# snap-research/GiGL

Measured on AMD Instinct MI355X. Metric: sampled+aggregated edges/s, higher is better.
Workload: dtype f32

## Files before the change

### gigl_amd/csrc/sample.hip

```cpp
#include "common.h"

#include <cstdlib>
#include <mutex>
#include <type_traits>

namespace {

constexpr uint64_t P1 = 0x9E3779B185EBCA87ULL;
constexpr uint64_t P2 = 0xC2B2AE3D27D4EB4FULL;
constexpr uint64_t P3 = 0x165667B19E3779F9ULL;
constexpr uint64_t P5 = 0x27D4EB2F165667C5ULL;
constexpr uint64_t SPARK_SEED = 42ULL;
constexpr uint64_t SIGN = 0x8000000000000000ULL;

__device__ __forceinline__ uint64_t xxh64_i32_ordered(uint32_t x) {
  uint64_t h = (SPARK_SEED + P5 + 4ULL) ^ ((uint64_t)x * P1);
  h = ((h << 23) | (h >> 41)) * P2 + P3;
  h ^= h >> 33;
  h *= P2;
  h ^= h >> 29;
  h *= P3;
  h ^= h >> 32;
  return h ^ SIGN;
}
// ... 373 lines not shown
    }
    return finish(count, lk, li);
  }
  __device__ __forceinline__ void serial(const RangeTable& tb, uint32_t n, uint32_t base, uint32_t T, bool in_table) {
    reset_best();
    if (!in_table) {
      scan_row(nullptr, (int64_t)n, base);
      return;
    }
    const uint32_t T4 = T >= (1u << 30) ? 0xFFFFFFFFu : 4u * T;
    const int l4 = T4 == 0xFFFFFFFFu ? 0 : min((int)__builtin_clz(T4 - 1u), tb.levels);
    if (l4 > 0) {
      if (scan_level(tb, l4, T4, n, base)) return;
      reset_best();
    }
    if constexpr (FAST) {
      scan_row(tb.flat, (int64_t)n, base);
      if (readlane32(idx, f - 1) == 0xFFFFFFFFu) tie = true;
    } else {
      scan_row(nullptr, (int64_t)n, base);
    }
  }
};

enum { ROW_INVALID = 0, ROW_COPY = 1, ROW_FLAT = 2, ROW_LEVEL = 3, ROW_HASH = 4, ROW_SERIAL = 5, ROW_SERIAL_HASH = 6,
       ROW_SKIP = 7 };

struct __attribute__((aligned(32))) RowDesc {
  int64_t s;
  uint32_t n;
  uint32_t base;
  uint32_t T;
  uint32_t kind_cnt;
  const void* ptr;
};

__device__ __forceinline__ float filter_lambda(int f) { return (float)f + 4.f * __builtin_sqrtf((float)f) + 4.f; }

constexpr int WORK_LISTS = 64;
constexpr int WORK_CNT_STRIDE = 32;

struct WorkLists {
  uint32_t* items;
  int32_t* count;
  int64_t cap;
  int32_t iters;
  int32_t wgs;
};

__host__ __device__ static inline int64_t work_list_cap(int64_t n_parents) {
  return ((n_parents / 256 + 1 + WORK_LISTS - 1) / WORK_LISTS) * 256;
}
static inline int64_t expand_desc_bytes(int64_t n_parents) {
  return (n_parents + 1) * (int64_t)sizeof(RowDesc) + WORK_LISTS * work_list_cap(n_parents) * 4 +
         WORK_LISTS * WORK_CNT_STRIDE * 4 + 512;
}

__global__ void work_counts_zero_kernel(int32_t* count) { count[threadIdx.x * WORK_CNT_STRIDE] = 0; }

__global__ __launch_bounds__(256) void plan_rows_kernel(ExpandArgs a, RangeTable tb, RowDesc* __restrict__ desc,
                                                        int64_t* heavy_list, int32_t* heavy_count, WorkLists wl) {
  __shared__ int32_t s_wave[4];
  __shared__ int32_t s_base;
  const uint32_t p = blockIdx.x * 256u + threadIdx.x;
  const int lane = threadIdx.x & 63, w = threadIdx.x >> 6;
  bool real = false;
  if (p <= (uint32_t)a.n_parents) {
    RowDesc d{};
    if (p == (uint32_t)a.n_parents) {
      d.kind_cnt = ROW_SKIP;
      desc[p] = d;
    } else {
      uint32_t v, ksum;
      parent_of(a, p, v, ksum);
      uint32_t* out = a.out_nbr + (int64_t)p * a.f;
      if (v == GIGL_INVALID || (int64_t)v >= a.n_nodes) {
        for (int j = 0; j < a.f; ++j) out[j] = GIGL_INVALID;
        a.out_cnt[p] = 0;
      } else {
        int64_t deg;
        if (a.peer_world) {
          const uint32_t q = v / a.peer_world, rk = v - q * a.peer_world;
          const int64_t* rp = a.peer_rowptr[rk];
          const int64_t s0 = rp[q];
          deg = rp[q + 1] - s0;
          d.s = ((int64_t)rk << 48) | s0;
        } else {
          d.s = a.rowptr[v];
          deg = a.rowptr[v + 1] - d.s;
        }
        d.n = (uint32_t)deg;
        d.base = ksum + (uint32_t)a.hash_add;
        if (deg <= a.f && !a.multi) {
          const uint32_t* row = row_of_desc(a, d.s);
          for (int j = 0; j < a.f; ++j) out[j] = j < (int)deg ? row[j] : GIGL_INVALID;
          a.out_cnt[p] = (int32_t)deg;
        } else if (deg <= a.f) {
          d.kind_cnt = ROW_COPY;
          desc[p] = d;
          real = true;
        } else {
          const bool in_table = (uint64_t)d.base + (uint64_t)deg < tb.dom;
          const float lam = filter_lambda(a.f);
          d.T = d.n <= 64u ? 0xFFFFFFFFu
                           : (uint32_t)fminf(lam * 4294967296.f * __builtin_amdgcn_rcpf((float)d.n), 4294967040.f);
          uint32_t kind;
          if (!in_table) {
            if (deg > HEAVY_DEG) {
              kind = ROW_SKIP;
              if (heavy_list) heavy_list[atomicAdd(heavy_count, 1)] = (int64_t)p;
            } else {
              kind = lam <= 56.f ? ROW_HASH : ROW_SERIAL_HASH;
            }
          } else if (lam > 56.f) {
            kind = ROW_SERIAL;
          } else {
            const int l = min((int)__builtin_clz(d.T - 1u), tb.levels);
            if (l == 0 || d.n <= (uint32_t)a.flat_max) {
              kind = ROW_FLAT;
              d.ptr = tb.flat;
            } else {
              const int gs = TBL_IDX_SHIFT + l;
              const uint32_t* off = tb.off[l];
              const uint32_t start = off[(d.base + 1u) >> gs], end = off[((d.base + d.n) >> gs) + 1u];
              if (end - start > 256u) {
                kind = ROW_SERIAL;
              } else {
                kind = ROW_LEVEL | ((end - start) << 3);
                d.ptr = tb.lvl[l] + start;
              }
            }
          }
          d.kind_cnt = kind;
          desc[p] = d;
          real = (kind & 7u) != ROW_SKIP;
        }
      }
    }
  }
  const unsigned long long m = __ballot(real);
  if (lane == 0) s_wave[w] = (int32_t)__popcll(m);
  __syncthreads();
  const int list = (int)(blockIdx.x % WORK_LISTS);
  if (threadIdx.x == 0) {
    const int32_t tot = s_wave[0] + s_wave[1] + s_wave[2] + s_wave[3];
    s_base = tot ? atomicAdd(&wl.count[list * WORK_CNT_STRIDE], tot) : 0;
  }
  __syncthreads();
  if (real) {
    int32_t pos = s_base + (int32_t)__popcll(m & ((1ull << lane) - 1ull));
    for (int k = 0; k < w; ++k) pos += s_wave[k];
    wl.items[(int64_t)list * wl.cap + pos] = p;
  }
}

struct Cand {
  uint32_t k0, j0, k1, j1;
  bool ahead;
};

__device__ __forceinline__ Cand fetch_candidates(const RowDesc& d, int lane) {
  Cand c;
  c.k0 = c.k1 = 0xFFFFFFFFu;
  c.j0 = c.j1 = d.base;
  c.ahead = false;
  const uint32_t kind = d.kind_cnt & 7u, cnt = d.kind_cnt >> 3;
  if (kind == ROW_LEVEL && cnt <= 128u) {
    const uint2* ent = (const uint2*)d.ptr;
    if ((uint32_t)lane < cnt) {
      const uint2 x = ent[lane];
      c.j0 = x.x;
      c.k0 = x.y;
    }
    if ((uint32_t)lane + 64u < cnt) {
      const uint2 x = ent[lane + 64];
      c.j1 = x.x;
      c.k1 = x.y;
    }
    c.ahead = true;
  } else if (kind == ROW_FLAT && d.n <= 128u) {
    const uint32_t* src = (const uint32_t*)d.ptr + d.base;
    c.j0 = d.base + (uint32_t)lane + 1u;
    c.k0 = src[lane + 1];
    if (d.n > 64u) {
      c.j1 = c.j0 + 64u;
      c.k1 = src[lane + 65];
    }
    c.ahead = true;
  }
  return c;
}

__device__ __forceinline__ bool select_ahead(Sel<true>& sel, const RowDesc& d, const Cand& c, uint32_t* lk, uint32_t* li) {
  const uint32_t n = d.n, T = d.T, base = d.base;
  const bool all = T == 0xFFFFFFFFu;
  uint32_t count = 0;
  const uint32_t i0 = c.j0 - base, i1 = c.j1 - base;
  sel.offer(c.k0 & sel.dmask, i0, (uint32_t)(i0 - 1u) < n && (all || c.k0 < T), count, lk, li);
  if ((d.kind_cnt & 7u) == ROW_LEVEL ? (d.kind_cnt >> 3) > 64u : n > 64u)
    sel.offer(c.k1 & sel.dmask, i1, (uint32_t)(i1 - 1u) < n && (all || c.k1 < T), count, lk, li);
  return sel.finish(count, lk, li);
}

__global__ __launch_bounds__(256) __attribute__((amdgpu_waves_per_eu(8, 8))) void expand_rows_kernel(
    ExpandArgs a, RangeTable tb, const RowDesc* __restrict__ desc, WorkLists wl) {
  __shared__ __attribute__((aligned(16))) uint32_t s_lk[4][72], s_li[4][64];
  const int lane = threadIdx.x & 63;
  const int wave_in_block = __builtin_amdgcn_readfirstlane((int)(threadIdx.x >> 6));
  const int f = a.f;
  uint32_t* lk = s_lk[wave_in_block];
  uint32_t* li = s_li[wave_in_block];
  const uint32_t wgs_p = wl.iters > 0 ? (uint32_t)wl.wgs : gridDim.x;
  const uint32_t round = blockIdx.x / wgs_p;
  const uint32_t gw = (blockIdx.x % wgs_p) * 4u + (uint32_t)wave_in_block, n_waves = wgs_p * 4u;
  const uint32_t list = gw % WORK_LISTS, stride = n_waves / WORK_LISTS;
  const int32_t n_items = __builtin_amdgcn_readfirstlane(wl.count[list * WORK_CNT_STRIDE]);
  const uint32_t* items = wl.items + (int64_t)list * wl.cap;
  const uint32_t k_first = gw / WORK_LISTS + stride * round * (uint32_t)wl.iters;
  const uint32_t k_end = wl.iters > 0 ? k_first + stride * (uint32_t)wl.iters : 0xFFFFFFFFu;
  for (uint32_t k = k_first; (int32_t)(2u * k) < n_items && k < k_end; k += stride) {
    const uint32_t p0 = __builtin_amdgcn_readfirstlane(items[2u * k]);
    const uint32_t p1 = (int32_t)(2u * k + 1u) < n_items ? __builtin_amdgcn_readfirstlane(items[2u * k + 1u])
                                                         : (uint32_t)a.n_parents;
    const RowDesc d0 = desc[p0], d1 = desc[p1];
    const Cand c0 = fetch_candidates(d0, lane), c1 = fetch_candidates(d1, lane);
    Sel<true> s0, s1;
    s0.init(f, lane, a.proxy_drop);
    s1.init(f, lane, a.proxy_drop);
    const bool done0 = c0.ahead && !a.multi && select_ahead(s0, d0, c0, lk, li) && !s0.tie;
    uint32_t slot0 = 0, val0 = 0;
    bool sel0 = false;
    if (done0) {
      const unsigned long long m = s0.selmask;
      sel0 = (m >> lane) & 1ull;
      slot0 = __builtin_amdgcn_mbcnt_hi((uint32_t)(m >> 32), __builtin_amdgcn_mbcnt_lo((uint32_t)m, 0u));
      if (sel0) val0 = row_of_desc(a, d0.s)[s0.idx - 1];
    }
    const bool done1 = c1.ahead && !a.multi && select_ahead(s1, d1, c1, lk, li) && !s1.tie;
    uint32_t slot1 = 0, val1 = 0;
    bool sel1 = false;
    if (done1) {
      const unsigned long long m = s1.selmask;
      sel1 = (m >> lane) & 1ull;
      slot1 = __builtin_amdgcn_mbcnt_hi((uint32_t)(m >> 32), __builtin_amdgcn_mbcnt_lo((uint32_t)m, 0u));
      if (sel1) val1 = row_of_desc(a, d1.s)[s1.idx - 1];
    }
    if (done0) {
      if (sel0) a.out_nbr[(int64_t)p0 * f + slot0] = val0;
      if (lane == 0) a.out_cnt[p0] = f;
    }
    if (done1) {
      if (sel1) a.out_nbr[(int64_t)p1 * f + slot1] = val1;
      if (lane == 0) a.out_cnt[p1] = f;
    }
    if (done0 && done1) continue;
  #pragma nounroll
    for (int r = 0; r < 2; ++r) {
      if (r == 0 ? done0 : done1) continue;
      const RowDesc d = r == 0 ? d0 : d1;
      const uint32_t p = r == 0 ? p0 : p1;
      const uint32_t kind = d.kind_cnt & 7u;
      if (kind == ROW_SKIP) continue;
      uint32_t* out = a.out_nbr + (int64_t)p * f;
      if (kind == ROW_INVALID) {
        if (lane < f) out[lane] = GIGL_INVALID;
        if (lane == 0) a.out_cnt[p] = 0;
        continue;
      }
      const uint32_t* row = row_of_desc(a, d.s);
      const uint32_t n = d.n, base = d.base, T = d.T;
      if (kind == ROW_COPY) {
        if (a.multi) {
          const int nw = emit_sorted_distinct(row, (uint32_t)lane < n ? (uint32_t)lane + 1u : 0xFFFFFFFFu, f, lane, out);
          if (lane == 0) a.out_cnt[p] = nw;
          continue;
        }
        if (lane < f) out[lane] = (uint32_t)lane < n ? row[lane] : GIGL_INVALID;
        if (lane == 0) a.out_cnt[p] = (int32_t)n;
        continue;
      }
      const bool in_table = kind != ROW_HASH && kind != ROW_SERIAL_HASH;
      uint32_t sel_idx;
      {
        Sel<true> fast;
        fast.init(f, lane, a.proxy_drop);
        bool done = false;
        if (kind == ROW_LEVEL) done = fast.filter_level((const uint2*)d.ptr, d.kind_cnt >> 3, n, T, base, lk, li);
        else if (kind == ROW_FLAT) done = fast.template filter_positions<SRC_FLAT>((const uint32_t*)d.ptr, n, T, base, lk, li);
        else if (kind == ROW_HASH) done = fast.template filter_positions<SRC_HASH>(nullptr, n, T, base, lk, li);
        if (!done) fast.serial(tb, n, base, T, in_table);
        sel_idx = fast.idx;
        if (fast.tie) {
          Sel<false> exact;
          exact.init(f, lane);
          exact.serial(tb, n, base, T, in_table);
          sel_idx = exact.idx;
        } else if (fast.ordered) {
          const unsigned long long m = fast.selmask;
          const bool sel = (m >> lane) & 1ull;
          const uint32_t slot = __builtin_amdgcn_mbcnt_hi((uint32_t)(m >> 32), __builtin_amdgcn_mbcnt_lo((uint32_t)m, 0u));
          const uint32_t val = sel ? row[sel_idx - 1] : GIGL_INVALID;
          if (!a.multi) {
            if (sel) out[slot] = val;
            if (lane == 0) a.out_cnt[p] = f;
            continue;
          }
          if (sel) lk[slot] = val;
          wave_lds_sync();
          const bool keep = sel && (slot == 0 || lk[slot - 1] != val);
          wave_lds_sync();
          const unsigned long long km = __ballot(keep);
          if (lane < f) out[lane] = GIGL_INVALID;
          if (keep) out[__builtin_amdgcn_mbcnt_hi((uint32_t)(km >> 32), __builtin_amdgcn_mbcnt_lo((uint32_t)km, 0u))] = val;
          if (lane == 0) a.out_cnt[p] = (int32_t)__popcll(km);
          continue;
        }
      }
      if (a.multi) {
        const int nw = emit_sorted_distinct(row, sel_idx, f, lane, out);
        if (lane == 0) a.out_cnt[p] = nw;
        continue;
      }
      emit_sorted(row, sel_idx, f, lane, out);
// ... 384 lines not shown
  e = hipMalloc(&own->mem2, bytes2);
  if (e != hipSuccess) {
    own->mem2 = nullptr;
    return fail_build(GIGL_E_OOM, "hipMalloc of the level lists failed", e);
  }
  RangeTable t{};
  t.dom = dom;
  t.levels = L;
  t.flat = flat;
  TableBuild tbuild{};
  tbuild.flat = flat;
  tbuild.tile_off = cnt;
  tbuild.total = total;
  tbuild.n_tiles = n_tiles;
  tbuild.levels = L;
  tbuild.dom = dom;
  for (int l = 1; l <= L; ++l) {
    tbuild.lvl[l] = (uint2*)((char*)own->mem2 + lvl_at[l]);
    tbuild.off[l] = (uint32_t*)(m0 + off_at[l]);
    t.lvl[l] = tbuild.lvl[l];
    t.off[l] = tbuild.off[l];
  }
  hipLaunchKernelGGL(table_fill_kernel, dim3(n_tiles), dim3(256), 0, ctx->stream, tbuild);
  e = hipGetLastError();
  if (e == hipSuccess) e = hipStreamSynchronize(ctx->stream);
  if (e != hipSuccess) return fail_build(GIGL_E_HIP, "filling failed", e);
  own->t = t;
  own->refs = 1;
  g_device_table[dev] = own;
  ctx->sampler_table = own;
  return GIGL_OK;
}

int32_t run_expand(gigl_ctx* ctx, const ExpandArgs& a_in, const RangeTable& tb, bool covered,
                   int64_t* heavy_list, int32_t* heavy_count, RowDesc* desc) {
  ExpandArgs a = a_in;
  if (a.f > GIGL_FAST_FANOUT) {
    gigl_prof_scope ps(ctx, GIGL_K_EXPAND);
    int64_t wgs = a.n_parents < 8192 ? a.n_parents : 8192;
    hipLaunchKernelGGL(expand_wide_kernel, dim3((unsigned)wgs), dim3(256), 0, ctx->stream, a);
    GIGL_HIP_CHECK(ctx, hipGetLastError());
    return GIGL_OK;
  }
  a.proxy_drop = 0;
  if (const char* e = getenv("GIGL_SAMPLER_PROXY_BITS")) {
    int bits = atoi(e);
    if (bits >= 1 && bits <= 32) a.proxy_drop = 32 - bits;
  }
  static const int32_t flat_max = [] {
    const char* e = getenv("GIGL_EXPAND_FLAT_MAX");
    return e ? atoi(e) : 128;
  }();
  a.flat_max = flat_max;
  if (!covered) gigl_fill_u32(ctx->stream, heavy_count, 0u, 1);
  WorkLists wl{};
  wl.cap = work_list_cap(a.n_parents);
  wl.items = reinterpret_cast<uint32_t*>(desc + a.n_parents + 1);
  wl.count = reinterpret_cast<int32_t*>(wl.items + (int64_t)WORK_LISTS * wl.cap);
  wl.count = reinterpret_cast<int32_t*>(((uintptr_t)wl.count + 127) & ~(uintptr_t)127);
  hipLaunchKernelGGL(work_counts_zero_kernel, dim3(1), dim3(WORK_LISTS), 0, ctx->stream, wl.count);
  {
    gigl_prof_scope ps(ctx, GIGL_K_EXPAND);
    hipLaunchKernelGGL(plan_rows_kernel, dim3((unsigned)(a.n_parents / 256 + 1)), dim3(256), 0, ctx->stream, a, tb,
                       desc, covered ? nullptr : heavy_list, heavy_count, wl);
    int64_t wgs = ((a.n_parents + 7) / 8 + 15) / 16 * 16;
    static const int64_t wgs_max = [] {
      const char* e = getenv("GIGL_EXPAND_WGS");
      const int64_t v = e ? atoll(e) : 2048;
      return v < 16 ? (int64_t)16 : v / 16 * 16;
    }();
    if (wgs > wgs_max) wgs = wgs_max;
    static const int32_t iters = [] {
      const char* e = getenv("GIGL_EXPAND_ITERS");
      const int v = e ? atoi(e) : 16;
      return v < 0 ? 0 : v;
    }();
    wl.iters = iters;
    wl.wgs = (int32_t)wgs;
    if (iters > 0) {
      const int64_t stride = wgs * 4 / WORK_LISTS;
      const int64_t steps = (wl.cap / 2 + stride - 1) / stride;
      wgs *= (steps + iters - 1) / iters;
    }
    hipLaunchKernelGGL(expand_rows_kernel, dim3((unsigned)wgs), dim3(256), 0, ctx->stream, a, tb, (const RowDesc*)desc, wl);
  }
  if (!covered) {
    gigl_prof_scope ps(ctx, GIGL_K_EXPAND_HEAVY);
    int64_t hb = a.n_parents < 2048 ? a.n_parents : 2048;
    hipLaunchKernelGGL(expand_heavy_kernel, dim3((unsigned)hb), dim3(256), 0, ctx->stream, a, heavy_list,
                       heavy_count);
  }
  GIGL_HIP_CHECK(ctx, hipGetLastError());
  return GIGL_OK;
}

uint64_t window_bound(const gigl_graph* g, int32_t hops, int32_t first_counter, int32_t sampling_seed) {
  uint64_t worst = 0;
  for (int k = 0; k < hops; ++k) {
    int64_t add = (int64_t)sampling_seed * (int64_t)(first_counter + k);
    if (add < 0 || add > (int64_t)0x7FFFFFFF) return ~0ULL;
    uint64_t hi = (uint64_t)(k + 1) * (uint64_t)(g->n > 0 ? g->n - 1 : 0) + (uint64_t)add + (uint64_t)g->maxdeg;
    if (hi > worst) worst = hi;
  }
  return worst;
}

__device__ __forceinline__ uint32_t mix32(uint32_t x) {
  x ^= x >> 16;
  x *= 0x7feb352dU;
  x ^= x >> 15;
  x *= 0x846ca68bU;
  x ^= x >> 16;
  return x;
}

__global__ __launch_bounds__(256) void expand_fast_kernel(ExpandArgs a) {
  const int lane = threadIdx.x & 63;
// ... 84 lines not shown
               "bad mode %d", mode);
  int64_t parents = b;
  for (int k = 0; k < hops; ++k) {
    if (fanouts[k] < 1 || fanouts[k] > GIGL_MAX_FANOUT)
      return gigl_fail(ctx, GIGL_E_UNSUPPORTED, "fanout[%d]=%d outside [1,%d]", k, fanouts[k],
                       GIGL_MAX_FANOUT);
    if (mode != GIGL_MODE_SPARK_HASH && fanouts[k] > GIGL_FAST_FANOUT)
      return gigl_fail(ctx, GIGL_E_UNSUPPORTED, "fanout[%d]=%d: the non-parity modes take fanouts up to %d", k, fanouts[k],
                       GIGL_FAST_FANOUT);
    GIGL_REQUIRE(ctx, out->nbr[k] && out->cnt[k], "tree buffers for hop %d are null", k);
    parents *= fanouts[k];
    GIGL_REQUIRE(ctx, parents < (int64_t)1 << 31, "tree too large");
  }
  GIGL_HIP_CHECK(ctx, hipSetDevice(ctx->device));
  out->hops = hops;
  out->b = b;
  for (int k = 0; k < hops; ++k) out->fanouts[k] = fanouts[k];
  if (b == 0) return GIGL_OK;

  RangeTable tb{};
  bool covered = false;
  int32_t rc = GIGL_OK;
  if (mode == GIGL_MODE_SPARK_HASH) {
    const uint64_t bound = window_bound(g, hops, 1, sampling_seed);
    const uint64_t cap = table_cap_j();
    rc = ensure_table(ctx, bound == ~0ULL ? (1ull << 20) : (bound + 1 < cap ? bound + 1 : cap));
    if (rc != GIGL_OK) return rc;
    tb = ((TableOwner*)ctx->sampler_table)->t;
    covered = bound != ~0ULL && bound < tb.dom;
  }

  int64_t* heavy_list = nullptr;
  int32_t* heavy_count = nullptr;
  RowDesc* desc = nullptr;
  if (mode == GIGL_MODE_SPARK_HASH) {
    int64_t max_parents = b, q = b;
    for (int k = 0; k + 1 < hops; ++k) {
      q *= fanouts[k];
      if (q > max_parents) max_parents = q;
    }
    rc = gigl_arena_reset(ctx, expand_desc_bytes(max_parents) + max_parents * 8 + 1024);
    if (rc != GIGL_OK) return rc;
    desc = (RowDesc*)gigl_arena_alloc(ctx, expand_desc_bytes(max_parents));
    if (!covered) {
      heavy_list = (int64_t*)gigl_arena_alloc(ctx, max_parents * 8);
      heavy_count = (int32_t*)gigl_arena_alloc(ctx, 256);
    }
    if (!desc || (!covered && (!heavy_list || !heavy_count))) return gigl_fail(ctx, GIGL_E_OOM, "arena exhausted");
  }

  ExpandArgs a{};
  a.rowptr = g->rowptr;
  a.col = g->col;
  a.n_nodes = g->n;
  a.multi = g->multi ? 1 : 0;
  a.roots = roots;
  parents = b;
  for (int k = 0; k < hops; ++k) {
    a.hop = k;
    a.n_parents = parents;
    a.f = fanouts[k];
    a.fan[k] = fanouts[k];
    a.hash_add = (int32_t)((uint32_t)sampling_seed * (uint32_t)(k + 1));
    a.out_nbr = out->nbr[k];
    a.out_cnt = out->cnt[k];
    if (mode == GIGL_MODE_FAST || mode == GIGL_MODE_REPLACE) {
      int64_t blocks = (parents + 3) / 4;
      if (blocks > 256 * 32) blocks = 256 * 32;
      gigl_prof_scope ps(ctx, GIGL_K_EXPAND);
      if (mode == GIGL_MODE_FAST)
        hipLaunchKernelGGL(expand_fast_kernel, dim3((unsigned)blocks), dim3(256), 0, ctx->stream, a);
      else
        hipLaunchKernelGGL(expand_replace_kernel, dim3((unsigned)blocks), dim3(256), 0, ctx->stream, a);
      GIGL_HIP_CHECK(ctx, hipGetLastError());
    } else {
      rc = run_expand(ctx, a, tb, covered, heavy_list, heavy_count, desc);
      if (rc != GIGL_OK) return rc;
    }
    a.anc[k] = out->nbr[k];
    parents *= fanouts[k];
  }
  return GIGL_OK;
}

int32_t gigl_sample_khop_peer(gigl_ctx* ctx, const int64_t* const* peer_rowptr, const uint32_t* const* peer_col,
                              int32_t world, int64_t n_global, int64_t max_window_end, const uint32_t* roots, int32_t b,
                              const int32_t* fanouts, int32_t hops, int32_t sampling_seed, gigl_tree* out) {
  if (!ctx) return GIGL_E_INVALID_ARG;
  GIGL_REQUIRE(ctx, peer_rowptr && peer_col && (roots || b == 0) && fanouts && out, "null argument");
  GIGL_REQUIRE(ctx, hops >= 1 && hops <= GIGL_MAX_HOPS && b >= 0 && world >= 1 && world < (1 << 15), "bad shape");
  int64_t parents = b, max_parents = b;
  for (int k = 0; k < hops; ++k) {
    if (fanouts[k] < 1 || fanouts[k] > GIGL_FAST_FANOUT)
      return gigl_fail(ctx, GIGL_E_UNSUPPORTED, "peer-mapped sampling takes fan-outs up to %d (fanout[%d]=%d)", GIGL_FAST_FANOUT, k,
                       fanouts[k]);
    GIGL_REQUIRE(ctx, out->nbr[k] && out->cnt[k], "tree buffers for hop %d are null", k);
    if (parents > max_parents) max_parents = parents;
    parents *= fanouts[k];
    GIGL_REQUIRE(ctx, parents < (int64_t)1 << 31, "tree too large");
  }
  GIGL_HIP_CHECK(ctx, hipSetDevice(ctx->device));
  out->hops = hops;
  out->b = b;
  for (int k = 0; k < hops; ++k) out->fanouts[k] = fanouts[k];
  if (b == 0) return GIGL_OK;
  const uint64_t cap = table_cap_j();
  if (max_window_end < 0 || (uint64_t)max_window_end + 1 > cap)
    return gigl_fail(ctx, GIGL_E_UNSUPPORTED, "peer-mapped sampling needs a window bound inside the threshold table (max_window_end)");
  int32_t rc = ensure_table(ctx, (uint64_t)max_window_end + 1);
  if (rc != GIGL_OK) return rc;
  const RangeTable tb = ((TableOwner*)ctx->sampler_table)->t;
  if ((uint64_t)max_window_end >= tb.dom)
    return gigl_fail(ctx, GIGL_E_UNSUPPORTED, "peer-mapped sampling: the window bound exceeds the threshold table");
  rc = gigl_arena_reset(ctx, expand_desc_bytes(max_parents) + 1024);
  if (rc != GIGL_OK) return rc;
  RowDesc* desc = (RowDesc*)gigl_arena_alloc(ctx, expand_desc_bytes(max_parents));
  if (!desc) return gigl_fail(ctx, GIGL_E_OOM, "arena exhausted");
  ExpandArgs a{};
  a.peer_rowptr = peer_rowptr;
  a.peer_col = peer_col;
  a.peer_world = (uint32_t)world;
  a.n_nodes = n_global;
  a.multi = 0;
  a.roots = roots;
  parents = b;
  for (int k = 0; k < hops; ++k) {
    a.hop = k;
    a.n_parents = parents;
    a.f = fanouts[k];
    a.fan[k] = fanouts[k];
    a.hash_add = (int32_t)((uint32_t)sampling_seed * (uint32_t)(k + 1));
    a.out_nbr = out->nbr[k];
    a.out_cnt = out->cnt[k];
    rc = run_expand(ctx, a, tb, true, nullptr, nullptr, desc);
    if (rc != GIGL_OK) return rc;
    a.anc[k] = out->nbr[k];
    parents *= fanouts[k];
  }
  return GIGL_OK;
}

int32_t gigl_expand_frontier(gigl_ctx* ctx, gigl_graph* shard, const uint32_t* nodes, const uint32_t* ksums,
                             int64_t m, int32_t f, int32_t hash_add, int32_t world, int64_t max_window_end,
                             uint32_t* out_nbr, int32_t* out_cnt) {
  if (!ctx) return GIGL_E_INVALID_ARG;
  GIGL_REQUIRE(ctx, shard && (m == 0 || (nodes && ksums && out_nbr && out_cnt)), "null argument");
  GIGL_REQUIRE(ctx, world >= 1 && m >= 0 && m < ((int64_t)1 << 31), "bad sizes");
  if (f < 1 || f > GIGL_MAX_FANOUT)
    return gigl_fail(ctx, GIGL_E_UNSUPPORTED, "fanout %d outside [1,%d]", f, GIGL_MAX_FANOUT);
  GIGL_HIP_CHECK(ctx, hipSetDevice(ctx->device));
  if (m == 0) return GIGL_OK;
  const uint64_t cap = table_cap_j();
  const bool bounded = max_window_end >= 0;
  const uint64_t bound = bounded ? (uint64_t)max_window_end : ~0ULL;
  int32_t rc = ensure_table(ctx, !bounded ? (1ull << 20) : (bound + 1 < cap ? bound + 1 : cap));
  if (rc != GIGL_OK) return rc;
  const RangeTable tb = ((TableOwner*)ctx->sampler_table)->t;
  const bool covered = bounded && bound < tb.dom;
  int64_t* heavy_list = nullptr;
  int32_t* heavy_count = nullptr;
  rc = gigl_arena_reset(ctx, expand_desc_bytes(m) + m * 8 + 1024);
  if (rc != GIGL_OK) return rc;
  RowDesc* desc = (RowDesc*)gigl_arena_alloc(ctx, expand_desc_bytes(m));
  if (!covered) {
    heavy_list = (int64_t*)gigl_arena_alloc(ctx, m * 8);
    heavy_count = (int32_t*)gigl_arena_alloc(ctx, 256);
  }
  if (!desc || (!covered && (!heavy_list || !heavy_count))) return gigl_fail(ctx, GIGL_E_OOM, "arena exhausted");
  ExpandArgs a{};
  a.rowptr = shard->rowptr;
  a.col = shard->col;
  a.n_nodes = shard->n;
  a.multi = shard->multi ? 1 : 0;
  a.hop = 0;
  a.n_parents = m;
  a.f = f;
  a.fan[0] = f;
  a.hash_add = hash_add;
  a.out_nbr = out_nbr;
  a.out_cnt = out_cnt;
  a.ex_nodes = nodes;
  a.ex_ksum = ksums;
  a.row_div = (uint32_t)world;
  return run_expand(ctx, a, tb, covered, heavy_list, heavy_count, desc);
}

int32_t gigl_sample_positives(gigl_ctx* ctx, gigl_graph* g_out, const uint32_t* roots, int32_t b,
                              int32_t f, int32_t sampling_seed, int32_t mode, uint32_t* pos,
                              int32_t* cnt) {
  return gigl_sample_out_neighbors(ctx, g_out, roots, b, f, sampling_seed, 3, mode, pos, cnt);
}

int32_t gigl_sample_out_neighbors(gigl_ctx* ctx, gigl_graph* g_out, const uint32_t* roots, int32_t b,
                                  int32_t f, int32_t sampling_seed, int32_t counter, int32_t mode, uint32_t* pos,
                                  int32_t* cnt) {
  if (!ctx) return GIGL_E_INVALID_ARG;
  GIGL_REQUIRE(ctx, counter >= 1 && counter <= 64, "permutation call counter %d outside [1,64]", counter);
  GIGL_REQUIRE(ctx, g_out && (roots || b == 0) && pos && cnt, "null argument");
  GIGL_REQUIRE(ctx, mode == GIGL_MODE_SPARK_HASH, "positives are parity-mode only");
  if (f < 1 || f > GIGL_MAX_FANOUT)
    return gigl_fail(ctx, GIGL_E_UNSUPPORTED, "num positives %d outside [1,%d]", f, GIGL_MAX_FANOUT);
  GIGL_HIP_CHECK(ctx, hipSetDevice(ctx->device));
  if (b == 0) return GIGL_OK;
  int32_t rc = gigl_arena_reset(ctx, expand_desc_bytes(b) + (int64_t)(b + 1) * 8 + 1024);
  if (rc != GIGL_OK) return rc;
  RowDesc* desc = (RowDesc*)gigl_arena_alloc(ctx, expand_desc_bytes(b));
  int64_t* heavy_list = (int64_t*)gigl_arena_alloc(ctx, (int64_t)b * 8);
  int32_t* heavy_count = (int32_t*)gigl_arena_alloc(ctx, 256);
  if (!desc || !heavy_list || !heavy_count) return gigl_fail(ctx, GIGL_E_OOM, "arena exhausted");
  ExpandArgs a{};
  a.rowptr = g_out->rowptr;
  a.col = g_out->col;
  a.n_nodes = g_out->n;
  a.multi = g_out->multi ? 1 : 0;
  a.roots = roots;
  a.hop = 0;
  a.n_parents = b;
  a.f = f;
  a.fan[0] = f;
  a.hash_add = (int32_t)((uint32_t)sampling_seed * (uint32_t)counter);
  a.out_nbr = pos;
  a.out_cnt = cnt;
  const uint64_t bound = window_bound(g_out, 1, counter, sampling_seed);
  const uint64_t cap = table_cap_j();
  rc = ensure_table(ctx, bound == ~0ULL ? (1ull << 20) : (bound + 1 < cap ? bound + 1 : cap));
  if (rc != GIGL_OK) return rc;
  const RangeTable tb = ((TableOwner*)ctx->sampler_table)->t;
  return run_expand(ctx, a, tb, bound != ~0ULL && bound < tb.dom, heavy_list, heavy_count, desc);
}

}
```

Before: 10.81 billion.

## Store full row descriptors in work lists and expand four rows per wave

The planner now writes the complete 32-byte row descriptor straight into the per-list work queue instead of a parent index that points into a separate descriptor array. The expand kernel loads four descriptors with a single coalesced 128-byte read and unpacks them with readlane, then batches candidate fetch, offer and finish across four rows to raise memory-level parallelism. Pointers in the descriptor are replaced by a level index and start offset. Work counters are zeroed once per call for all hops instead of by one launch per hop. The costs are more LDS per wave, higher register pressure under the fixed waves-per-EU, and fewer work-groups because each wave now handles more rows.

```diff
diff --git a/gigl_amd/csrc/sample.hip b/gigl_amd/csrc/sample.hip
--- a/gigl_amd/csrc/sample.hip
+++ b/gigl_amd/csrc/sample.hip
@@ -429,16 +429,26 @@
   uint32_t base;
   uint32_t T;
   uint32_t kind_cnt;
-  const void* ptr;
+  uint32_t start;
+  uint32_t p;
 };
+static_assert(sizeof(RowDesc) == 32, "four descriptors are one 128-byte run: dword i in lane i");
+enum { RD_S_LO = 0, RD_S_HI = 1, RD_N = 2, RD_BASE = 3, RD_T = 4, RD_KIND = 5, RD_START = 6, RD_P = 7 };
+
+__device__ __forceinline__ uint32_t desc_kind(uint32_t kind_cnt) { return kind_cnt & 7u; }
+__device__ __forceinline__ uint32_t desc_level(uint32_t kind_cnt) { return (kind_cnt >> 3) & 31u; }
+__device__ __forceinline__ uint32_t desc_cnt(uint32_t kind_cnt) { return kind_cnt >> 8; }
 
 __device__ __forceinline__ float filter_lambda(int f) { return (float)f + 4.f * __builtin_sqrtf((float)f) + 4.f; }
 
 constexpr int WORK_LISTS = 64;
 constexpr int WORK_CNT_STRIDE = 32;
+constexpr int EXPAND_ROWS = 4;
+constexpr int64_t WORK_CNT_BYTES = (int64_t)GIGL_MAX_HOPS * WORK_LISTS * WORK_CNT_STRIDE * 4;
+static_assert(WORK_CNT_BYTES % 256 == 0, "the lists behind the counters keep the scratch's alignment");
 
 struct WorkLists {
-  uint32_t* items;
+  RowDesc* desc;
   int32_t* count;
   int64_t cap;
   int32_t iters;
@@ -449,89 +459,83 @@
   return ((n_parents / 256 + 1 + WORK_LISTS - 1) / WORK_LISTS) * 256;
 }
 static inline int64_t expand_desc_bytes(int64_t n_parents) {
-  return (n_parents + 1) * (int64_t)sizeof(RowDesc) + WORK_LISTS * work_list_cap(n_parents) * 4 +
-         WORK_LISTS * WORK_CNT_STRIDE * 4 + 512;
-}
-
-__global__ void work_counts_zero_kernel(int32_t* count) { count[threadIdx.x * WORK_CNT_STRIDE] = 0; }
-
-__global__ __launch_bounds__(256) void plan_rows_kernel(ExpandArgs a, RangeTable tb, RowDesc* __restrict__ desc,
-                                                        int64_t* heavy_list, int32_t* heavy_count, WorkLists wl) {
+  return WORK_CNT_BYTES + WORK_LISTS * work_list_cap(n_parents) * (int64_t)sizeof(RowDesc) + 512;
+}
+
+__global__ void work_counts_zero_kernel(int32_t* count) {
+  count[(blockIdx.x * WORK_LISTS + threadIdx.x) * WORK_CNT_STRIDE] = 0;
+}
+
+__global__ __launch_bounds__(256) void plan_rows_kernel(ExpandArgs a, RangeTable tb, int64_t* heavy_list,
+                                                        int32_t* heavy_count, WorkLists wl) {
   __shared__ int32_t s_wave[4];
   __shared__ int32_t s_base;
   const uint32_t p = blockIdx.x * 256u + threadIdx.x;
   const int lane = threadIdx.x & 63, w = threadIdx.x >> 6;
   bool real = false;
-  if (p <= (uint32_t)a.n_parents) {
-    RowDesc d{};
-    if (p == (uint32_t)a.n_parents) {
-      d.kind_cnt = ROW_SKIP;
-      desc[p] = d;
+  RowDesc d{};
+  d.p = p;
+  if (p < (uint32_t)a.n_parents) {
+    uint32_t v, ksum;
+    parent_of(a, p, v, ksum);
+    uint32_t* out = a.out_nbr + (int64_t)p * a.f;
+    if (v == GIGL_INVALID || (int64_t)v >= a.n_nodes) {
+      for (int j = 0; j < a.f; ++j) out[j] = GIGL_INVALID;
+      a.out_cnt[p] = 0;
     } else {
-      uint32_t v, ksum;
-      parent_of(a, p, v, ksum);
-      uint32_t* out = a.out_nbr + (int64_t)p * a.f;
-      if (v == GIGL_INVALID || (int64_t)v >= a.n_nodes) {
-        for (int j = 0; j < a.f; ++j) out[j] = GIGL_INVALID;
-        a.out_cnt[p] = 0;
+      int64_t deg;
+      if (a.peer_world) {
+        const uint32_t q = v / a.peer_world, rk = v - q * a.peer_world;
+        const int64_t* rp = a.peer_rowptr[rk];
+        const int64_t s0 = rp[q];
+        deg = rp[q + 1] - s0;
+        d.s = ((int64_t)rk << 48) | s0;
       } else {
-        int64_t deg;
-        if (a.peer_world) {
-          const uint32_t q = v / a.peer_world, rk = v - q * a.peer_world;
-          const int64_t* rp = a.peer_rowptr[rk];
-          const int64_t s0 = rp[q];
-          deg = rp[q + 1] - s0;
-          d.s = ((int64_t)rk << 48) | s0;
+        d.s = a.rowptr[v];
+        deg = a.rowptr[v + 1] - d.s;
+      }
+      d.n = (uint32_t)deg;
+      d.base = ksum + (uint32_t)a.hash_add;
+      if (deg <= a.f && !a.multi) {
+        const uint32_t* row = row_of_desc(a, d.s);
+        for (int j = 0; j < a.f; ++j) out[j] = j < (int)deg ? row[j] : GIGL_INVALID;
+        a.out_cnt[p] = (int32_t)deg;
+      } else if (deg <= a.f) {
+        d.kind_cnt = ROW_COPY;
+        real = true;
+      } else {
+        const bool in_table = (uint64_t)d.base + (uint64_t)deg < tb.dom;
+        const float lam = filter_lambda(a.f);
+        d.T = d.n <= 64u ? 0xFFFFFFFFu
+                         : (uint32_t)fminf(lam * 4294967296.f * __builtin_amdgcn_rcpf((float)d.n), 4294967040.f);
+        uint32_t kind;
+        if (!in_table) {
+          if (deg > HEAVY_DEG) {
+            kind = ROW_SKIP;
+            if (heavy_list) heavy_list[atomicAdd(heavy_count, 1)] = (int64_t)p;
+          } else {
+            kind = lam <= 56.f ? ROW_HASH : ROW_SERIAL_HASH;
+          }
+        } else if (lam > 56.f) {
+          kind = ROW_SERIAL;
         } else {
-          d.s = a.rowptr[v];
-          deg = a.rowptr[v + 1] - d.s;
-        }
-        d.n = (uint32_t)deg;
-        d.base = ksum + (uint32_t)a.hash_add;
-        if (deg <= a.f && !a.multi) {
-          const uint32_t* row = row_of_desc(a, d.s);
-          for (int j = 0; j < a.f; ++j) out[j] = j < (int)deg ? row[j] : GIGL_INVALID;
-          a.out_cnt[p] = (int32_t)deg;
-        } else if (deg <= a.f) {
-          d.kind_cnt = ROW_COPY;
-          desc[p] = d;
-          real = true;
-        } else {
-          const bool in_table = (uint64_t)d.base + (uint64_t)deg < tb.dom;
-          const float lam = filter_lambda(a.f);
-          d.T = d.n <= 64u ? 0xFFFFFFFFu
-                           : (uint32_t)fminf(lam * 4294967296.f * __builtin_amdgcn_rcpf((float)d.n), 4294967040.f);
-          uint32_t kind;
-          if (!in_table) {
-            if (deg > HEAVY_DEG) {
-              kind = ROW_SKIP;
-              if (heavy_list) heavy_list[atomicAdd(heavy_count, 1)] = (int64_t)p;
+          const int l = min((int)__builtin_clz(d.T - 1u), tb.levels);
+          if (l == 0 || d.n <= (uint32_t)a.flat_max) {
+            kind = ROW_FLAT;
+          } else {
+            const int gs = TBL_IDX_SHIFT + l;
+            const uint32_t* off = tb.off[l];
+            const uint32_t start = off[(d.base + 1u) >> gs], end = off[((d.base + d.n) >> gs) + 1u];
+            if (end - start > 256u) {
+              kind = ROW_SERIAL;
             } else {
-              kind = lam <= 56.f ? ROW_HASH : ROW_SERIAL_HASH;
-            }
-          } else if (lam > 56.f) {
-            kind = ROW_SERIAL;
-          } else {
-            const int l = min((int)__builtin_clz(d.T - 1u), tb.levels);
-            if (l == 0 || d.n <= (uint32_t)a.flat_max) {
-              kind = ROW_FLAT;
-              d.ptr = tb.flat;
-            } else {
-              const int gs = TBL_IDX_SHIFT + l;
-              const uint32_t* off = tb.off[l];
-              const uint32_t start = off[(d.base + 1u) >> gs], end = off[((d.base + d.n) >> gs) + 1u];
-              if (end - start > 256u) {
-                kind = ROW_SERIAL;
-              } else {
-                kind = ROW_LEVEL | ((end - start) << 3);
-                d.ptr = tb.lvl[l] + start;
-              }
+              kind = ROW_LEVEL | ((uint32_t)l << 3) | ((end - start) << 8);
+              d.start = start;
             }
           }
-          d.kind_cnt = kind;
-          desc[p] = d;
-          real = (kind & 7u) != ROW_SKIP;
         }
+        d.kind_cnt = kind;
+        real = (kind & 7u) != ROW_SKIP;
       }
     }
   }
@@ -547,116 +551,136 @@
   if (real) {
     int32_t pos = s_base + (int32_t)__popcll(m & ((1ull << lane) - 1ull));
     for (int k = 0; k < w; ++k) pos += s_wave[k];
-    wl.items[(int64_t)list * wl.cap + pos] = p;
+    wl.desc[(int64_t)list * wl.cap + pos] = d;
   }
 }
 
 struct Cand {
-  uint32_t k0, j0, k1, j1;
-  bool ahead;
+  uint32_t a0, k0, a1, k1;
 };
 
-__device__ __forceinline__ Cand fetch_candidates(const RowDesc& d, int lane) {
+__device__ __forceinline__ bool fetched_ahead(uint32_t kind_cnt, uint32_t n) {
+  const uint32_t kind = desc_kind(kind_cnt);
+  return (kind == ROW_LEVEL && desc_cnt(kind_cnt) <= 128u) || (kind == ROW_FLAT && n <= 128u);
+}
+__device__ __forceinline__ uint32_t ahead_items(uint32_t kind_cnt, uint32_t n) {
+  if (!fetched_ahead(kind_cnt, n)) return 0u;
+  return desc_kind(kind_cnt) == ROW_LEVEL ? desc_cnt(kind_cnt) : n;
+}
+
+__device__ __forceinline__ const uint2* level_run(const RangeTable& tb, const RowDesc& d) {
+  return tb.lvl[desc_level(d.kind_cnt)] + d.start;
+}
+
+__device__ __forceinline__ RowDesc desc_of_lanes(uint32_t dv, uint32_t r) {
+  const int l0 = (int)(r * 8u);
+  RowDesc d;
+  d.s = (int64_t)(((uint64_t)readlane32(dv, l0 + RD_S_HI) << 32) | readlane32(dv, l0 + RD_S_LO));
+  d.n = readlane32(dv, l0 + RD_N);
+  d.base = readlane32(dv, l0 + RD_BASE);
+  d.T = readlane32(dv, l0 + RD_T);
+  d.kind_cnt = readlane32(dv, l0 + RD_KIND);
+  d.start = readlane32(dv, l0 + RD_START);
+  d.p = readlane32(dv, l0 + RD_P);
+  return d;
+}
+
+__device__ __forceinline__ Cand fetch_candidates(const RangeTable& tb, const RowDesc& d, int lane) {
+  const bool lvl = desc_kind(d.kind_cnt) == ROW_LEVEL;
+  const uint32_t items = ahead_items(d.kind_cnt, d.n);
+  const uint32_t* run = items == 0u ? tb.flat : lvl ? reinterpret_cast<const uint32_t*>(level_run(tb, d)) : tb.flat + d.base;
+  const uint32_t shift = lvl ? 1u : 0u;
   Cand c;
-  c.k0 = c.k1 = 0xFFFFFFFFu;
-  c.j0 = c.j1 = d.base;
-  c.ahead = false;
-  const uint32_t kind = d.kind_cnt & 7u, cnt = d.kind_cnt >> 3;
-  if (kind == ROW_LEVEL && cnt <= 128u) {
-    const uint2* ent = (const uint2*)d.ptr;
-    if ((uint32_t)lane < cnt) {
-      const uint2 x = ent[lane];
-      c.j0 = x.x;
-      c.k0 = x.y;
-    }
-    if ((uint32_t)lane + 64u < cnt) {
-      const uint2 x = ent[lane + 64];
-      c.j1 = x.x;
-      c.k1 = x.y;
-    }
-    c.ahead = true;
-  } else if (kind == ROW_FLAT && d.n <= 128u) {
-    const uint32_t* src = (const uint32_t*)d.ptr + d.base;
-    c.j0 = d.base + (uint32_t)lane + 1u;
-    c.k0 = src[lane + 1];
-    if (d.n > 64u) {
-      c.j1 = c.j0 + 64u;
-      c.k1 = src[lane + 65];
-    }
-    c.ahead = true;
+  const uint32_t l0 = (uint32_t)lane < items ? (uint32_t)lane : 0u;
+  const uint32_t* q0 = run + (l0 << shift);
+  c.a0 = q0[0];
+  c.k0 = q0[1];
+  c.a1 = c.k1 = 0u;
+  if (items > 64u) {
+    const uint32_t l1 = (uint32_t)lane + 64u < items ? (uint32_t)lane + 64u : 0u;
+    const uint32_t* q1 = run + (l1 << shift);
+    c.a1 = q1[0];
+    c.k1 = q1[1];
   }
   return c;
 }
 
-__device__ __forceinline__ bool select_ahead(Sel<true>& sel, const RowDesc& d, const Cand& c, uint32_t* lk, uint32_t* li) {
+__device__ __forceinline__ uint32_t offer_ahead(Sel<true>& sel, const RowDesc& d, const Cand& c, int lane, uint32_t* lk, uint32_t* li) {
   const uint32_t n = d.n, T = d.T, base = d.base;
-  const bool all = T == 0xFFFFFFFFu;
+  const bool all = T == 0xFFFFFFFFu, lvl = desc_kind(d.kind_cnt) == ROW_LEVEL;
+  const uint32_t items = ahead_items(d.kind_cnt, n);
   uint32_t count = 0;
-  const uint32_t i0 = c.j0 - base, i1 = c.j1 - base;
-  sel.offer(c.k0 & sel.dmask, i0, (uint32_t)(i0 - 1u) < n && (all || c.k0 < T), count, lk, li);
-  if ((d.kind_cnt & 7u) == ROW_LEVEL ? (d.kind_cnt >> 3) > 64u : n > 64u)
-    sel.offer(c.k1 & sel.dmask, i1, (uint32_t)(i1 - 1u) < n && (all || c.k1 < T), count, lk, li);
-  return sel.finish(count, lk, li);
+  const uint32_t i0 = lvl ? c.a0 - base : (uint32_t)lane + 1u, i1 = lvl ? c.a1 - base : (uint32_t)lane + 65u;
+  sel.offer(c.k0 & sel.dmask, i0, (uint32_t)lane < items && (uint32_t)(i0 - 1u) < n && (all || c.k0 < T), count, lk, li);
+  if (items > 64u)
+    sel.offer(c.k1 & sel.dmask, i1, (uint32_t)lane + 64u < items && (uint32_t)(i1 - 1u) < n && (all || c.k1 < T), count, lk, li);
+  return count;
 }
 
 __global__ __launch_bounds__(256) __attribute__((amdgpu_waves_per_eu(8, 8))) void expand_rows_kernel(
-    ExpandArgs a, RangeTable tb, const RowDesc* __restrict__ desc, WorkLists wl) {
-  __shared__ __attribute__((aligned(16))) uint32_t s_lk[4][72], s_li[4][64];
+    ExpandArgs a, RangeTable tb, WorkLists wl) {
+  __shared__ __attribute__((aligned(16))) uint32_t s_lk[4][EXPAND_ROWS][72], s_li[4][EXPAND_ROWS][64];
   const int lane = threadIdx.x & 63;
   const int wave_in_block = __builtin_amdgcn_readfirstlane((int)(threadIdx.x >> 6));
   const int f = a.f;
-  uint32_t* lk = s_lk[wave_in_block];
-  uint32_t* li = s_li[wave_in_block];
+  uint32_t* lk = s_lk[wave_in_block][0];
+  uint32_t* li = s_li[wave_in_block][0];
   const uint32_t wgs_p = wl.iters > 0 ? (uint32_t)wl.wgs : gridDim.x;
   const uint32_t round = blockIdx.x / wgs_p;
   const uint32_t gw = (blockIdx.x % wgs_p) * 4u + (uint32_t)wave_in_block, n_waves = wgs_p * 4u;
   const uint32_t list = gw % WORK_LISTS, stride = n_waves / WORK_LISTS;
   const int32_t n_items = __builtin_amdgcn_readfirstlane(wl.count[list * WORK_CNT_STRIDE]);
-  const uint32_t* items = wl.items + (int64_t)list * wl.cap;
+  const uint32_t* words = reinterpret_cast<const uint32_t*>(wl.desc + (int64_t)list * wl.cap);
   const uint32_t k_first = gw / WORK_LISTS + stride * round * (uint32_t)wl.iters;
   const uint32_t k_end = wl.iters > 0 ? k_first + stride * (uint32_t)wl.iters : 0xFFFFFFFFu;
-  for (uint32_t k = k_first; (int32_t)(2u * k) < n_items && k < k_end; k += stride) {
-    const uint32_t p0 = __builtin_amdgcn_readfirstlane(items[2u * k]);
-    const uint32_t p1 = (int32_t)(2u * k + 1u) < n_items ? __builtin_amdgcn_readfirstlane(items[2u * k + 1u])
-                                                         : (uint32_t)a.n_parents;
-    const RowDesc d0 = desc[p0], d1 = desc[p1];
-    const Cand c0 = fetch_candidates(d0, lane), c1 = fetch_candidates(d1, lane);
-    Sel<true> s0, s1;
-    s0.init(f, lane, a.proxy_drop);
-    s1.init(f, lane, a.proxy_drop);
-    const bool done0 = c0.ahead && !a.multi && select_ahead(s0, d0, c0, lk, li) && !s0.tie;
-    uint32_t slot0 = 0, val0 = 0;
-    bool sel0 = false;
-    if (done0) {
-      const unsigned long long m = s0.selmask;
-      sel0 = (m >> lane) & 1ull;
-      slot0 = __builtin_amdgcn_mbcnt_hi((uint32_t)(m >> 32), __builtin_amdgcn_mbcnt_lo((uint32_t)m, 0u));
-      if (sel0) val0 = row_of_desc(a, d0.s)[s0.idx - 1];
-    }
-    const bool done1 = c1.ahead && !a.multi && select_ahead(s1, d1, c1, lk, li) && !s1.tie;
-    uint32_t slot1 = 0, val1 = 0;
-    bool sel1 = false;
-    if (done1) {
-      const unsigned long long m = s1.selmask;
-      sel1 = (m >> lane) & 1ull;
-      slot1 = __builtin_amdgcn_mbcnt_hi((uint32_t)(m >> 32), __builtin_amdgcn_mbcnt_lo((uint32_t)m, 0u));
-      if (sel1) val1 = row_of_desc(a, d1.s)[s1.idx - 1];
-    }
-    if (done0) {
-      if (sel0) a.out_nbr[(int64_t)p0 * f + slot0] = val0;
-      if (lane == 0) a.out_cnt[p0] = f;
-    }
-    if (done1) {
-      if (sel1) a.out_nbr[(int64_t)p1 * f + slot1] = val1;
-      if (lane == 0) a.out_cnt[p1] = f;
-    }
-    if (done0 && done1) continue;
+  for (uint32_t k = k_first; (int32_t)(EXPAND_ROWS * k) < n_items && k < k_end; k += stride) {
+    const uint32_t rows = min((uint32_t)n_items - EXPAND_ROWS * k, (uint32_t)EXPAND_ROWS);
+    const uint32_t dv = words[(uint64_t)k * (EXPAND_ROWS * 8u) + ((uint32_t)lane & 31u)];
+    Cand c[EXPAND_ROWS];
+#pragma unroll
+    for (uint32_t r = 0; r < EXPAND_ROWS; ++r) {
+      RowDesc d = desc_of_lanes(dv, r);
+      if (r >= rows) d.kind_cnt = ROW_INVALID;
+      c[r] = fetch_candidates(tb, d, lane);
+    }
+    Sel<true> s[EXPAND_ROWS];
+    uint32_t fast = 0, done = 0, count[EXPAND_ROWS], val[EXPAND_ROWS];
+#pragma unroll
+    for (uint32_t r = 0; r < EXPAND_ROWS; ++r) {
+      s[r].init(f, lane, a.proxy_drop);
+      count[r] = 0;
+      const RowDesc d = desc_of_lanes(dv, r);
+      if (r < rows && !a.multi && fetched_ahead(d.kind_cnt, d.n)) {
+        fast |= 1u << r;
+        count[r] = offer_ahead(s[r], d, c[r], lane, s_lk[wave_in_block][r], s_li[wave_in_block][r]);
+      }
+    }
+#pragma unroll
+    for (uint32_t r = 0; r < EXPAND_ROWS; ++r) {
+      val[r] = 0;
+      if (((fast >> r) & 1u) && s[r].finish(count[r], s_lk[wave_in_block][r], s_li[wave_in_block][r]) && !s[r].tie) {
+        done |= 1u << r;
+        if ((s[r].selmask >> lane) & 1ull)
+          val[r] = row_of_desc(a, desc_of_lanes(dv, r).s)[s[r].idx - 1];
+      }
+    }
+#pragma unroll
+    for (uint32_t r = 0; r < EXPAND_ROWS; ++r) {
+      if ((done >> r) & 1u) {
+        const uint32_t p = readlane32(dv, (int)(r * 8u) + RD_P);
+        const unsigned long long m = s[r].selmask;
+        const uint32_t slot = __builtin_amdgcn_mbcnt_hi((uint32_t)(m >> 32), __builtin_amdgcn_mbcnt_lo((uint32_t)m, 0u));
+        if ((m >> lane) & 1ull) a.out_nbr[(int64_t)p * f + slot] = val[r];
+        if (lane == 0) a.out_cnt[p] = f;
+      }
+    }
+    if (done == (1u << rows) - 1u) continue;
   #pragma nounroll
-    for (int r = 0; r < 2; ++r) {
-      if (r == 0 ? done0 : done1) continue;
-      const RowDesc d = r == 0 ? d0 : d1;
-      const uint32_t p = r == 0 ? p0 : p1;
-      const uint32_t kind = d.kind_cnt & 7u;
+    for (uint32_t r = 0; r < rows; ++r) {
+      if ((done >> r) & 1u) continue;
+      const RowDesc d = desc_of_lanes(dv, r);
+      const uint32_t p = d.p;
+      const uint32_t kind = desc_kind(d.kind_cnt);
       if (kind == ROW_SKIP) continue;
       uint32_t* out = a.out_nbr + (int64_t)p * f;
       if (kind == ROW_INVALID) {
@@ -681,11 +705,11 @@
       {
         Sel<true> fast;
         fast.init(f, lane, a.proxy_drop);
-        bool done = false;
-        if (kind == ROW_LEVEL) done = fast.filter_level((const uint2*)d.ptr, d.kind_cnt >> 3, n, T, base, lk, li);
-        else if (kind == ROW_FLAT) done = fast.template filter_positions<SRC_FLAT>((const uint32_t*)d.ptr, n, T, base, lk, li);
-        else if (kind == ROW_HASH) done = fast.template filter_positions<SRC_HASH>(nullptr, n, T, base, lk, li);
-        if (!done) fast.serial(tb, n, base, T, in_table);
+        bool done_row = false;
+        if (kind == ROW_LEVEL) done_row = fast.filter_level(level_run(tb, d), desc_cnt(d.kind_cnt), n, T, base, lk, li);
+        else if (kind == ROW_FLAT) done_row = fast.template filter_positions<SRC_FLAT>(tb.flat, n, T, base, lk, li);
+        else if (kind == ROW_HASH) done_row = fast.template filter_positions<SRC_HASH>(nullptr, n, T, base, lk, li);
+        if (!done_row) fast.serial(tb, n, base, T, in_table);
         sel_idx = fast.idx;
         if (fast.tie) {
           Sel<false> exact;
@@ -1136,8 +1160,12 @@
   return GIGL_OK;
 }
 
+void zero_work_counts(gigl_ctx* ctx, void* scratch, int sets) {
+  hipLaunchKernelGGL(work_counts_zero_kernel, dim3((unsigned)sets), dim3(WORK_LISTS), 0, ctx->stream, (int32_t*)scratch);
+}
+
 int32_t run_expand(gigl_ctx* ctx, const ExpandArgs& a_in, const RangeTable& tb, bool covered,
-                   int64_t* heavy_list, int32_t* heavy_count, RowDesc* desc) {
+                   int64_t* heavy_list, int32_t* heavy_count, void* scratch, int cset) {
   ExpandArgs a = a_in;
   if (a.f > GIGL_FAST_FANOUT) {
     gigl_prof_scope ps(ctx, GIGL_K_EXPAND);
@@ -1159,15 +1187,13 @@
   if (!covered) gigl_fill_u32(ctx->stream, heavy_count, 0u, 1);
   WorkLists wl{};
   wl.cap = work_list_cap(a.n_parents);
-  wl.items = reinterpret_cast<uint32_t*>(desc + a.n_parents + 1);
-  wl.count = reinterpret_cast<int32_t*>(wl.items + (int64_t)WORK_LISTS * wl.cap);
-  wl.count = reinterpret_cast<int32_t*>(((uintptr_t)wl.count + 127) & ~(uintptr_t)127);
-  hipLaunchKernelGGL(work_counts_zero_kernel, dim3(1), dim3(WORK_LISTS), 0, ctx->stream, wl.count);
+  wl.count = reinterpret_cast<int32_t*>(scratch) + (int64_t)cset * WORK_LISTS * WORK_CNT_STRIDE;
+  wl.desc = reinterpret_cast<RowDesc*>(reinterpret_cast<char*>(scratch) + WORK_CNT_BYTES);
   {
     gigl_prof_scope ps(ctx, GIGL_K_EXPAND);
     hipLaunchKernelGGL(plan_rows_kernel, dim3((unsigned)(a.n_parents / 256 + 1)), dim3(256), 0, ctx->stream, a, tb,
-                       desc, covered ? nullptr : heavy_list, heavy_count, wl);
-    int64_t wgs = ((a.n_parents + 7) / 8 + 15) / 16 * 16;
+                       covered ? nullptr : heavy_list, heavy_count, wl);
+    int64_t wgs = ((a.n_parents + 4 * EXPAND_ROWS - 1) / (4 * EXPAND_ROWS) + 15) / 16 * 16;
     static const int64_t wgs_max = [] {
       const char* e = getenv("GIGL_EXPAND_WGS");
       const int64_t v = e ? atoll(e) : 2048;
@@ -1183,10 +1209,10 @@
     wl.wgs = (int32_t)wgs;
     if (iters > 0) {
       const int64_t stride = wgs * 4 / WORK_LISTS;
-      const int64_t steps = (wl.cap / 2 + stride - 1) / stride;
+      const int64_t steps = (wl.cap / EXPAND_ROWS + stride - 1) / stride;
       wgs *= (steps + iters - 1) / iters;
     }
-    hipLaunchKernelGGL(expand_rows_kernel, dim3((unsigned)wgs), dim3(256), 0, ctx->stream, a, tb, (const RowDesc*)desc, wl);
+    hipLaunchKernelGGL(expand_rows_kernel, dim3((unsigned)wgs), dim3(256), 0, ctx->stream, a, tb, wl);
   }
   if (!covered) {
     gigl_prof_scope ps(ctx, GIGL_K_EXPAND_HEAVY);
@@ -1337,7 +1363,7 @@
 
   int64_t* heavy_list = nullptr;
   int32_t* heavy_count = nullptr;
-  RowDesc* desc = nullptr;
+  void* desc = nullptr;
   if (mode == GIGL_MODE_SPARK_HASH) {
     int64_t max_parents = b, q = b;
     for (int k = 0; k + 1 < hops; ++k) {
@@ -1346,12 +1372,13 @@
     }
     rc = gigl_arena_reset(ctx, expand_desc_bytes(max_parents) + max_parents * 8 + 1024);
     if (rc != GIGL_OK) return rc;
-    desc = (RowDesc*)gigl_arena_alloc(ctx, expand_desc_bytes(max_parents));
+    desc = gigl_arena_alloc(ctx, expand_desc_bytes(max_parents));
     if (!covered) {
       heavy_list = (int64_t*)gigl_arena_alloc(ctx, max_parents * 8);
       heavy_count = (int32_t*)gigl_arena_alloc(ctx, 256);
     }
     if (!desc || (!covered && (!heavy_list || !heavy_count))) return gigl_fail(ctx, GIGL_E_OOM, "arena exhausted");
+    zero_work_counts(ctx, desc, hops);
   }
 
   ExpandArgs a{};
@@ -1379,7 +1406,7 @@
         hipLaunchKernelGGL(expand_replace_kernel, dim3((unsigned)blocks), dim3(256), 0, ctx->stream, a);
       GIGL_HIP_CHECK(ctx, hipGetLastError());
     } else {
-      rc = run_expand(ctx, a, tb, covered, heavy_list, heavy_count, desc);
+      rc = run_expand(ctx, a, tb, covered, heavy_list, heavy_count, desc, k);
       if (rc != GIGL_OK) return rc;
     }
     a.anc[k] = out->nbr[k];
@@ -1419,8 +1446,9 @@
     return gigl_fail(ctx, GIGL_E_UNSUPPORTED, "peer-mapped sampling: the window bound exceeds the threshold table");
   rc = gigl_arena_reset(ctx, expand_desc_bytes(max_parents) + 1024);
   if (rc != GIGL_OK) return rc;
-  RowDesc* desc = (RowDesc*)gigl_arena_alloc(ctx, expand_desc_bytes(max_parents));
+  void* desc = gigl_arena_alloc(ctx, expand_desc_bytes(max_parents));
   if (!desc) return gigl_fail(ctx, GIGL_E_OOM, "arena exhausted");
+  zero_work_counts(ctx, desc, hops);
   ExpandArgs a{};
   a.peer_rowptr = peer_rowptr;
   a.peer_col = peer_col;
@@ -1437,7 +1465,7 @@
     a.hash_add = (int32_t)((uint32_t)sampling_seed * (uint32_t)(k + 1));
     a.out_nbr = out->nbr[k];
     a.out_cnt = out->cnt[k];
-    rc = run_expand(ctx, a, tb, true, nullptr, nullptr, desc);
+    rc = run_expand(ctx, a, tb, true, nullptr, nullptr, desc, k);
     if (rc != GIGL_OK) return rc;
     a.anc[k] = out->nbr[k];
     parents *= fanouts[k];
@@ -1466,12 +1494,13 @@
   int32_t* heavy_count = nullptr;
   rc = gigl_arena_reset(ctx, expand_desc_bytes(m) + m * 8 + 1024);
   if (rc != GIGL_OK) return rc;
-  RowDesc* desc = (RowDesc*)gigl_arena_alloc(ctx, expand_desc_bytes(m));
+  void* desc = gigl_arena_alloc(ctx, expand_desc_bytes(m));
   if (!covered) {
     heavy_list = (int64_t*)gigl_arena_alloc(ctx, m * 8);
     heavy_count = (int32_t*)gigl_arena_alloc(ctx, 256);
   }
   if (!desc || (!covered && (!heavy_list || !heavy_count))) return gigl_fail(ctx, GIGL_E_OOM, "arena exhausted");
+  zero_work_counts(ctx, desc, 1);
   ExpandArgs a{};
   a.rowptr = shard->rowptr;
   a.col = shard->col;
@@ -1487,7 +1516,7 @@
   a.ex_nodes = nodes;
   a.ex_ksum = ksums;
   a.row_div = (uint32_t)world;
-  return run_expand(ctx, a, tb, covered, heavy_list, heavy_count, desc);
+  return run_expand(ctx, a, tb, covered, heavy_list, heavy_count, desc, 0);
 }
 
 int32_t gigl_sample_positives(gigl_ctx* ctx, gigl_graph* g_out, const uint32_t* roots, int32_t b,
@@ -1509,10 +1538,11 @@
   if (b == 0) return GIGL_OK;
   int32_t rc = gigl_arena_reset(ctx, expand_desc_bytes(b) + (int64_t)(b + 1) * 8 + 1024);
   if (rc != GIGL_OK) return rc;
-  RowDesc* desc = (RowDesc*)gigl_arena_alloc(ctx, expand_desc_bytes(b));
+  void* desc = gigl_arena_alloc(ctx, expand_desc_bytes(b));
   int64_t* heavy_list = (int64_t*)gigl_arena_alloc(ctx, (int64_t)b * 8);
   int32_t* heavy_count = (int32_t*)gigl_arena_alloc(ctx, 256);
   if (!desc || !heavy_list || !heavy_count) return gigl_fail(ctx, GIGL_E_OOM, "arena exhausted");
+  zero_work_counts(ctx, desc, 1);
   ExpandArgs a{};
   a.rowptr = g_out->rowptr;
   a.col = g_out->col;
@@ -1531,7 +1561,7 @@
   rc = ensure_table(ctx, bound == ~0ULL ? (1ull << 20) : (bound + 1 < cap ? bound + 1 : cap));
   if (rc != GIGL_OK) return rc;
   const RangeTable tb = ((TableOwner*)ctx->sampler_table)->t;
-  return run_expand(ctx, a, tb, bound != ~0ULL && bound < tb.dom, heavy_list, heavy_count, desc);
-}
-
-}
+  return run_expand(ctx, a, tb, bound != ~0ULL && bound < tb.dom, heavy_list, heavy_count, desc, 0);
+}
+
+}
```

Result: slower. 10.69 billion (-1.2%).
